# PKU-Alignment/SafeVLA

Hardware: AMD Instinct MI355X
Metric: env-steps/sec through PPO-Lagrangian update (higher is better)
Workload: dtype bf16

## Files before the change

safevla_amd/csrc/attn.hip:

```cpp
#include "attn_host.h"

#define HD 64
#define ATT_THREADS 256

struct AttnArgs {
    const bf16_t *Q, *K, *V; long ld;
    bf16_t* O; long ldo;
    float* LSE;
    const bf16_t* dO; long lddo;
    bf16_t *dQ, *dK, *dV; long ldd;
    const int* traj;
    const float* bias;
    const unsigned char* kvalid;
    int S, H, mask_mode;
    float scale;
    int kv_rows;
    int Sq;
    long ldq, lddq;
    float* Dws;
    DropCfg drop;
    int xcd_rows;
};

template <int SP, int THREADS = ATT_THREADS>
__device__ __forceinline__ void stage_head(bf16_t* dst, const bf16_t* src, long ld, int S, int tid) {
    constexpr int IT = SP * 8 / THREADS;
    u32x4 w[IT];
#pragma unroll
    for (int i = 0; i < IT; ++i) {
        const int q = tid + i * THREADS;
        const int row = q >> 3, c = q & 7;
        w[i] = u32x4{0, 0, 0, 0};
        if (row < S) w[i] = *(const u32x4*)(src + (size_t)row * ld + c * 8);
    }
#pragma unroll
    for (int i = 0; i < IT; ++i) {
        const int q = tid + i * THREADS;
        *(u32x4*)(dst + (q >> 3) * LDSROW + (((q & 7) ^ att_swz(q >> 3)) << 3)) = w[i];
    }
}

template <int NKT, bool GENERIC, int NW = 4, bool EXACT = false>
__device__ __forceinline__ void attn_fwd_kernel_body(AttnArgs p) {
    p.drop = drop_resolve(p.drop);
    extern __shared__ __attribute__((aligned(16))) char smem[];
    constexpr int SP = NKT * 16;
    bf16_t* Ks = (bf16_t*)smem;
    bf16_t* Vs = Ks + SP * LDSROW;
    int* traj_s = (int*)(Vs + SP * LDSROW);
    unsigned char* kv_s = (unsigned char*)(traj_s + SP);
    const int tid = threadIdx.x, lane = tid & 63, wid = tid >> 6;
    const int r = blockIdx.x / p.H, h = blockIdx.x % p.H;
    const size_t tok0 = (size_t)r * p.kv_rows, mtok0 = (size_t)r * p.S;
    const int S = p.S;
    stage_head<SP, NW * 64>(Ks, p.K + tok0 * p.ld + h * HD, p.ld, S, tid);
    stage_head<SP, NW * 64>(Vs, p.V + tok0 * p.ld + h * HD, p.ld, S, tid);
    for (int i = tid; i < SP; i += NW * 64) {
        traj_s[i] = (p.traj && i < S) ? p.traj[mtok0 + i] : -1;
        kv_s[i] = (p.kvalid && i < S) ? p.kvalid[mtok0 + i] : 1;
    }
    const int ql = lane & 15, g = lane >> 4;
    const int Sq = p.Sq;
    const size_t qtok0 = (size_t)r * Sq;
    const int nqt = (Sq + 15) / 16;
    constexpr int MAXQT = (NKT + NW - 1) / NW;
    bf16x8 qall[MAXQT][2];
#pragma unroll
    for (int t = 0; t < MAXQT; ++t) {
        const int q = (wid + NW * t) * 16 + ql;
        const bool ok = q < Sq;
        const bf16_t* qp = p.Q + (qtok0 + (ok ? q : 0)) * p.ldq + h * HD + 8 * g;
        qall[t][0] = ok ? *(const bf16x8*)qp : bf16x8{0, 0, 0, 0, 0, 0, 0, 0};
        qall[t][1] = ok ? *(const bf16x8*)(qp + 32) : bf16x8{0, 0, 0, 0, 0, 0, 0, 0};
    }
    __syncthreads();
    const unsigned char* kvp = p.kvalid ? kv_s : nullptr;
    const RowBase Krow = att_row_base(Ks, lane);
    const TrBase Vtr = att_tr_base(Vs, lane);
#pragma unroll
    for (int t = 0; t < MAXQT; ++t) {
        const int qt = wid + NW * t;
        if (qt >= nqt) break;
        const int q = qt * 16 + ql;
        const bf16x8 qf[2] = {qall[t][0], qall[t][1]};
        float sc[NKT][4];
        float mx = -INFINITY;
        const float sl2 = p.scale * LOG2E;
#pragma unroll
        for (int kt = 0; kt < NKT; ++kt) {
            f32x4 a = {0.f, 0.f, 0.f, 0.f};
            if (EXACT || kt * 16 < S) {
                a = mfma16(lds_row8i(Krow.lo, kt * 16), qf[0], a);
                a = mfma16(lds_row8i(Krow.hi, kt * 16), qf[1], a);
            }
            if constexpr (GENERIC) {
#pragma unroll
                for (int e = 0; e < 4; ++e) {
                    const int key = kt * 16 + 4 * g + e;
                    float s = a[e] * p.scale;
                    if (p.bias && q < Sq && key < S) s += p.bias[((size_t)h * S + q) * S + key];
                    s *= LOG2E;
                    if (att_masked(p, q < Sq ? q : 0, key, traj_s, kvp)) s = -INFINITY;
                    sc[kt][e] = s;
                    mx = fmaxf(mx, s);
                }
            } else {
                const bool tail = EXACT ? kt >= NKT - 2 : (kt + 1) * 16 > S;
#pragma unroll
                for (int e = 0; e < 4; ++e) {
                    float s = a[e] * sl2;
                    if (tail && kt * 16 + 4 * g + e >= S) s = -INFINITY;
                    sc[kt][e] = s;
                    mx = fmaxf(mx, s);
                }
            }
        }
        mx = fmaxf(mx, __shfl_xor(mx, 16, 64));
        mx = fmaxf(mx, __shfl_xor(mx, 32, 64));
        if (mx == -INFINITY) mx = 0.f;
        float lsum = 0.f;
#pragma unroll
        for (int kt = 0; kt < NKT; ++kt)
#pragma unroll
            for (int e = 0; e < 4; ++e) { sc[kt][e] = __builtin_amdgcn_exp2f(sc[kt][e] - mx); lsum += sc[kt][e]; }
        lsum += __shfl_xor(lsum, 16, 64);
        lsum += __shfl_xor(lsum, 32, 64);
        if (p.drop.thr) {
            const unsigned long long rb = att_drop_row(p.S, p.H, r, h, q < Sq ? q : 0);
#pragma unroll
            for (int kt = 0; kt < NKT; ++kt) {
                const unsigned keep = drop_keep4(p.drop, rb + kt * 16 + 4 * g);
#pragma unroll
                for (int e = 0; e < 4; ++e) if (!((keep >> e) & 1u)) sc[kt][e] = 0.f;
            }
        }
        f32x4 o[4];
#pragma unroll
        for (int dt = 0; dt < 4; ++dt) o[dt] = f32x4{0.f, 0.f, 0.f, 0.f};
#pragma unroll
        for (int u = 0; u < NKT / 2; ++u) {
            if (EXACT || u * 32 < S) {
                const float pv[8] = {sc[2 * u][0], sc[2 * u][1], sc[2 * u][2], sc[2 * u][3],
                                     sc[2 * u + 1][0], sc[2 * u + 1][1], sc[2 * u + 1][2], sc[2 * u + 1][3]};
                const bf16x8 pa = pack8(pv);
#pragma unroll
                for (int dt = 0; dt < 4; ++dt)
                    o[dt] = mfma16(lds_tr8i(Vtr.d[dt], 32 * u, 32 * u + 16), pa, o[dt]);
            }
        }
        const float inv = lsum > 0.f ? p.drop.scale / lsum : 0.f;
        if (q < Sq) {
#pragma unroll
            for (int dt = 0; dt < 4; ++dt) {
                const u32x2 w = {pack_bf2(o[dt][0] * inv, o[dt][1] * inv), pack_bf2(o[dt][2] * inv, o[dt][3] * inv)};
                *(u32x2*)(p.O + (qtok0 + q) * p.ldo + h * HD + dt * 16 + 4 * g) = w;
            }
        }
        if (p.LSE && g == 0 && q < Sq) p.LSE[((size_t)r * p.H + h) * Sq + q] = (mx + __log2f(lsum)) * LN2;
    }
}

__device__ __forceinline__ void att_xcd_item(const AttnArgs& p, int item, int nitems, int& r, int& h) {
    if (!p.xcd_rows) return;
    const int x = item & 7, j = item >> 3, nfull = (nitems / 64) * 8;
    if ((j >> 3) * 8 + x < nfull) { r = (j >> 3) * 8 + x; h = j & 7; }
}
struct AttDrop {
    unsigned a0;
    unsigned hb;
    bool wrap;
    unsigned long long p0;
};
__device__ __forceinline__ AttDrop att_drop_head(const AttnArgs& p, int r, int h) {
    AttDrop d;
    d.p0 = att_drop_row(p.S, p.H, r, h, 0) >> 1;
    d.a0 = (unsigned)d.p0 * 0x9E3779B1u;
    d.hb = ((unsigned)(d.p0 >> 32) * 0x85EBCA77u) ^ p.drop.key;
    d.wrap = (unsigned)d.p0 > 0xFFFF0000u;
    return d;
}

template <int NKT>
__device__ __forceinline__ void attn_fwd_persist_kernel_body(AttnArgs p, int nitems) {
    p.drop = drop_resolve(p.drop);
    extern __shared__ __attribute__((aligned(16))) char smem[];
    constexpr int SP = NKT * 16, IT = SP * 8 / ATT_THREADS, MAXQT = (NKT + 3) / 4;
    bf16_t* Ks = (bf16_t*)smem;
    bf16_t* Vs = Ks + SP * LDSROW;
    const int tid = threadIdx.x, lane = tid & 63, wid = tid >> 6;
    const int ql = lane & 15, g = lane >> 4;
    const int S = p.S, Sq = p.Sq, nqt = (Sq + 15) / 16;
    u32x4 kreg[IT], vreg[IT];
    bf16x8 qreg[MAXQT][2];
    auto fetch = [&](int item) {
        int r = item / p.H, h = item % p.H;
        att_xcd_item(p, item, nitems, r, h);
        const bf16_t* kp = p.K + (size_t)r * p.kv_rows * p.ld + h * HD;
        const bf16_t* vp = p.V + (size_t)r * p.kv_rows * p.ld + h * HD;
#pragma unroll
        for (int i = 0; i < IT; ++i) {
            const int q = tid + i * ATT_THREADS, row = q >> 3, c = q & 7;
            kreg[i] = u32x4{0, 0, 0, 0}; vreg[i] = u32x4{0, 0, 0, 0};
            if (row < S) {
                kreg[i] = *(const u32x4*)(kp + (size_t)row * p.ld + c * 8);
                vreg[i] = *(const u32x4*)(vp + (size_t)row * p.ld + c * 8);
            }
        }
#pragma unroll
        for (int t = 0; t < MAXQT; ++t) {
            const int q = (wid + 4 * t) * 16 + ql;
            const bool ok = q < Sq;
            const bf16_t* qp = p.Q + ((size_t)r * Sq + (ok ? q : 0)) * p.ldq + h * HD + 8 * g;
            qreg[t][0] = ok ? *(const bf16x8*)qp : bf16x8{0, 0, 0, 0, 0, 0, 0, 0};
            qreg[t][1] = ok ? *(const bf16x8*)(qp + 32) : bf16x8{0, 0, 0, 0, 0, 0, 0, 0};
        }
    };
    int item = blockIdx.x;
    if (item >= nitems) return;
    fetch(item);
    const RowBase Krow = att_row_base(Ks, lane);
    const TrBase Vtr = att_tr_base(Vs, lane);
    const float sl2 = p.scale * LOG2E;
    for (; item < nitems; item += gridDim.x) {
        int r = item / p.H, h = item % p.H;
        att_xcd_item(p, item, nitems, r, h);
        const size_t qtok0 = (size_t)r * Sq;
        __syncthreads();
#pragma unroll
        for (int i = 0; i < IT; ++i) {
            const int q = tid + i * ATT_THREADS;
            const int off = (q >> 3) * LDSROW + (((q & 7) ^ att_swz(q >> 3)) << 3);
            *(u32x4*)(Ks + off) = kreg[i];
            *(u32x4*)(Vs + off) = vreg[i];
        }
        bf16x8 qcur[MAXQT][2];
#pragma unroll
        for (int t = 0; t < MAXQT; ++t) { qcur[t][0] = qreg[t][0]; qcur[t][1] = qreg[t][1]; }
        __syncthreads();
        if (item + (int)gridDim.x < nitems) fetch(item + gridDim.x);
#pragma unroll
        for (int t = 0; t < MAXQT; ++t) {
            const int qt = wid + 4 * t;
            if (qt >= nqt) break;
            const int q = qt * 16 + ql;
            f32x4 sc[NKT];
            f32x4 mx4 = {-INFINITY, -INFINITY, -INFINITY, -INFINITY};
#pragma unroll
            for (int kt = 0; kt < NKT; ++kt) {
                f32x4 a = {0.f, 0.f, 0.f, 0.f};
                a = mfma16(lds_row8i(Krow.lo, kt * 16), qcur[t][0], a);
                a = mfma16(lds_row8i(Krow.hi, kt * 16), qcur[t][1], a);
                if (kt >= NKT - 2) {
#pragma unroll
                    for (int e = 0; e < 4; ++e)
                        if (kt * 16 + 4 * g + e >= S) a[e] = -INFINITY;
                }
                sc[kt] = a;
                mx4 = __builtin_elementwise_max(mx4, a);
            }
            float mx = fmaxf(fmaxf(mx4[0], mx4[1]), fmaxf(mx4[2], mx4[3]));
            mx = fmaxf(mx, __shfl_xor(mx, 16, 64));
            mx = fmaxf(mx, __shfl_xor(mx, 32, 64));
            const float nm = -mx * sl2;
            const f32x4 nm4 = {nm, nm, nm, nm}, sl4 = {sl2, sl2, sl2, sl2};
            f32x4 ls4 = {0.f, 0.f, 0.f, 0.f};
#pragma unroll
            for (int kt = 0; kt < NKT; ++kt) {
                const f32x4 x = sc[kt] * sl4 + nm4;
#pragma unroll
                for (int e = 0; e < 4; ++e) sc[kt][e] = __builtin_amdgcn_exp2f(x[e]);
                ls4 += sc[kt];
            }
            float lsum = (ls4[0] + ls4[1]) + (ls4[2] + ls4[3]);
            lsum += __shfl_xor(lsum, 16, 64);
            lsum += __shfl_xor(lsum, 32, 64);
            if (p.drop.thr) {
                const AttDrop dh = att_drop_head(p, r, h);
                const int S4 = (S + 3) & ~3, hS = S4 >> 1;
                const unsigned thr = p.drop.thr;
                if (!dh.wrap) {
                    const unsigned al = dh.a0 + (unsigned)(ql * hS + 2 * g) * 0x9E3779B1u;
                    const unsigned uq = (unsigned)(qt * 16 * hS) * 0x9E3779B1u;
#pragma unroll
                    for (int kt = 0; kt < NKT; ++kt) {
                        const unsigned ub = uq + (unsigned)(kt * 8) * 0x9E3779B1u;
                        const unsigned r0 = drop_mix((al + ub) ^ dh.hb), r1 = drop_mix((al + ub + 0x9E3779B1u) ^ dh.hb);
                        if ((r0 & 0xffffu) < thr) sc[kt][0] = 0.f;
                        if ((r0 >> 16) < thr) sc[kt][1] = 0.f;
                        if ((r1 & 0xffffu) < thr) sc[kt][2] = 0.f;
                        if ((r1 >> 16) < thr) sc[kt][3] = 0.f;
                    }
                } else {
                    const unsigned long long rb = att_drop_row(p.S, p.H, r, h, q < Sq ? q : 0);
#pragma unroll
                    for (int kt = 0; kt < NKT; ++kt) {
                        const unsigned keep = drop_keep4(p.drop, rb + kt * 16 + 4 * g);
#pragma unroll
                        for (int e = 0; e < 4; ++e) if (!((keep >> e) & 1u)) sc[kt][e] = 0.f;
                    }
                }
            }
            f32x4 o[4];
#pragma unroll
            for (int dt = 0; dt < 4; ++dt) o[dt] = f32x4{0.f, 0.f, 0.f, 0.f};
#pragma unroll
            for (int u = 0; u < NKT / 2; ++u) {
                const float pv[8] = {sc[2 * u][0], sc[2 * u][1], sc[2 * u][2], sc[2 * u][3],
                                     sc[2 * u + 1][0], sc[2 * u + 1][1], sc[2 * u + 1][2], sc[2 * u + 1][3]};
                const bf16x8 pa = pack8(pv);
#pragma unroll
                for (int dt = 0; dt < 4; ++dt)
                    o[dt] = mfma16(lds_tr8i(Vtr.d[dt], 32 * u, 32 * u + 16), pa, o[dt]);
            }
            const float inv = lsum > 0.f ? p.drop.scale / lsum : 0.f;
            if (q < Sq) {
#pragma unroll
                for (int dt = 0; dt < 4; ++dt) {
                    const u32x2 w = {pack_bf2(o[dt][0] * inv, o[dt][1] * inv), pack_bf2(o[dt][2] * inv, o[dt][3] * inv)};
                    *(u32x2*)(p.O + (qtok0 + q) * p.ldo + h * HD + dt * 16 + 4 * g) = w;
                }
            }
            if (p.LSE && g == 0 && q < Sq) p.LSE[((size_t)r * p.H + h) * Sq + q] = (mx * sl2 + __log2f(lsum)) * LN2;
        }
    }
}


template <int NKT, bool GENERIC>
__global__ void __launch_bounds__(ATT_THREADS) attn_bwd_dq_kernel(AttnArgs p) {
    p.drop = drop_resolve(p.drop);
    extern __shared__ __attribute__((aligned(16))) char smem[];
    constexpr int SP = NKT * 16;
    bf16_t* Ks = (bf16_t*)smem;
    bf16_t* Vs = Ks + SP * LDSROW;
    int* traj_s = (int*)(Vs + SP * LDSROW);
    unsigned char* kv_s = (unsigned char*)(traj_s + SP);
    const int tid = threadIdx.x, lane = tid & 63, wid = tid >> 6;
    const int r = blockIdx.x / p.H, h = blockIdx.x % p.H;
    const size_t tok0 = (size_t)r * p.S;
    const int S = p.S;
    stage_head<SP>(Ks, p.K + tok0 * p.ld + h * HD, p.ld, S, tid);
    stage_head<SP>(Vs, p.V + tok0 * p.ld + h * HD, p.ld, S, tid);
    for (int i = tid; i < SP; i += ATT_THREADS) {
        traj_s[i] = (p.traj && i < S) ? p.traj[tok0 + i] : -1;
        kv_s[i] = (p.kvalid && i < S) ? p.kvalid[tok0 + i] : 1;
    }
    const int ql = lane & 15, g = lane >> 4;
    const int Sq = p.Sq;
    const size_t qtok0 = (size_t)r * Sq;
    constexpr int MAXQT = (NKT + 3) / 4;
    bf16x8 qall[MAXQT][4];
    float dall[MAXQT], lall[MAXQT];
#pragma unroll
    for (int t = 0; t < MAXQT; ++t) {
        const int q = (wid + 4 * t) * 16 + ql;
        const bool qok = q < Sq;
        const bf16_t* qp = p.Q + (qtok0 + (qok ? q : 0)) * p.ldq + h * HD + 8 * g;
        const bf16_t* gp = p.dO + (qtok0 + (qok ? q : 0)) * p.lddo + h * HD + 8 * g;
        const bf16_t* op = p.O + (qtok0 + (qok ? q : 0)) * p.ldo + h * HD + 8 * g;
        qall[t][0] = gld8(qp, qok); qall[t][1] = gld8(qp + 32, qok);
        qall[t][2] = gld8(gp, qok); qall[t][3] = gld8(gp + 32, qok);
        dall[t] = dot8(qall[t][2], gld8(op, qok)) + dot8(qall[t][3], gld8(op + 32, qok));
        lall[t] = qok ? p.LSE[((size_t)r * p.H + h) * Sq + q] : INFINITY;
    }
    __syncthreads();
    const unsigned char* kvp = p.kvalid ? kv_s : nullptr;
    const RowBase Krow = att_row_base(Ks, lane), Vrow = att_row_base(Vs, lane);
    const TrBase Ktr = att_tr_base(Ks, lane);
    const int ntile = (Sq + 15) / 16;
#pragma unroll
    for (int t = 0; t < MAXQT; ++t) {
        const int qt = wid + 4 * t;
        if (qt >= ntile) break;
        const int q = qt * 16 + ql;
        const bool qok = q < Sq;
        const bf16x8 qf0 = qall[t][0], qf1 = qall[t][1], gf0 = qall[t][2], gf1 = qall[t][3];
        float D_q = dall[t];
        D_q += __shfl_xor(D_q, 16, 64);
        D_q += __shfl_xor(D_q, 32, 64);
        const float lse_q = lall[t];
        const float sl2 = p.scale * LOG2E, lse2_q = lse_q * LOG2E;
        f32x4 dq[4];
#pragma unroll
        for (int dt = 0; dt < 4; ++dt) dq[dt] = f32x4{0.f, 0.f, 0.f, 0.f};
#pragma unroll
        for (int u = 0; u < NKT / 2; ++u) {
            if (u * 32 < S) {
                float dsv[8];
#pragma unroll
                for (int e2 = 0; e2 < 2; ++e2) {
                    const int kt = 2 * u + e2;
                    f32x4 s = {0.f, 0.f, 0.f, 0.f}, dp = {0.f, 0.f, 0.f, 0.f};
                    s = mfma16(lds_row8i(Krow.lo, kt * 16), qf0, s);
                    s = mfma16(lds_row8i(Krow.hi, kt * 16), qf1, s);
                    dp = mfma16(lds_row8i(Vrow.lo, kt * 16), gf0, dp);
                    dp = mfma16(lds_row8i(Vrow.hi, kt * 16), gf1, dp);
                    const unsigned dkeep = p.drop.thr ? drop_keep4(p.drop, att_drop_row(p.S, p.H, r, h, qok ? q : 0) + kt * 16 + 4 * g) : 0xfu;
                    if constexpr (GENERIC) {
#pragma unroll
                        for (int e = 0; e < 4; ++e) {
                            const int key = kt * 16 + 4 * g + e;
                            float sv = s[e] * p.scale;
                            if (p.bias && qok && key < S) sv += p.bias[((size_t)h * S + q) * S + key];
                            const bool mk = !qok || att_masked(p, qok ? q : 0, key, traj_s, kvp);
                            const float pr = mk ? 0.f : __expf(sv - lse_q);
                            dsv[e2 * 4 + e] = pr * (((dkeep >> e) & 1u ? dp[e] * p.drop.scale : 0.f) - D_q) * p.scale;
                        }
                    } else {
#pragma unroll
                        for (int e = 0; e < 4; ++e)
                            dsv[e2 * 4 + e] = __builtin_amdgcn_exp2f(s[e] * sl2 - lse2_q) * (((dkeep >> e) & 1u ? dp[e] * p.drop.scale : 0.f) - D_q) * p.scale;
                    }
                }
                const bf16x8 da = pack8(dsv);
#pragma unroll
                for (int dt = 0; dt < 4; ++dt)
                    dq[dt] = mfma16(lds_tr8i(Ktr.d[dt], 32 * u, 32 * u + 16), da, dq[dt]);
            }
        }
        if (qok) {
#pragma unroll
            for (int dt = 0; dt < 4; ++dt) {
                const u32x2 w = {pack_bf2(dq[dt][0], dq[dt][1]), pack_bf2(dq[dt][2], dq[dt][3])};
                *(u32x2*)(p.dQ + (qtok0 + q) * p.lddq + h * HD + dt * 16 + 4 * g) = w;
            }
        }
    }
}

template <int NKT, bool GENERIC>
__global__ void __launch_bounds__(ATT_THREADS, NKT <= 12 ? 3 : 1) attn_bwd_dkv_kernel(AttnArgs p) {
    p.drop = drop_resolve(p.drop);
    extern __shared__ __attribute__((aligned(16))) char smem[];
    constexpr int SP = NKT * 16;
    bf16_t* Qs = (bf16_t*)smem;
    bf16_t* Gs = Qs + SP * LDSROW;
    float* lse_s = (float*)(Gs + SP * LDSROW);
    float* D_s = lse_s + SP;
    int* traj_s = (int*)(D_s + SP);
    unsigned char* kv_s = (unsigned char*)(traj_s + SP);
    const int tid = threadIdx.x, lane = tid & 63, wid = tid >> 6;
    const int r = blockIdx.x / p.H, h = blockIdx.x % p.H;
    const size_t tok0 = (size_t)r * p.S;
    const int S = p.S;
    constexpr int MAXKT = (NKT + 3) / 4;
    bf16x8 kvbuf[2][4];
    auto load_kv = [&](int t, bf16x8 (&dst)[4]) {
        const int keyl = (wid + 4 * t) * 16 + (lane & 15);
        const bool kok = keyl < S;
        const bf16_t* kp = p.K + (tok0 + (kok ? keyl : 0)) * p.ld + h * HD + 8 * (lane >> 4);
        const bf16_t* vp = p.V + (tok0 + (kok ? keyl : 0)) * p.ld + h * HD + 8 * (lane >> 4);
        dst[0] = gld8(kp, kok); dst[1] = gld8(kp + 32, kok);
        dst[2] = gld8(vp, kok); dst[3] = gld8(vp + 32, kok);
    };
    load_kv(0, kvbuf[0]);
    const int Sq = p.Sq;
    const size_t qtok0 = (size_t)r * Sq;
    stage_head<SP>(Qs, p.Q + qtok0 * p.ldq + h * HD, p.ldq, Sq, tid);
    stage_head<SP>(Gs, p.dO + qtok0 * p.lddo + h * HD, p.lddo, Sq, tid);
    for (int i = tid; i < SP; i += ATT_THREADS) {
        traj_s[i] = (p.traj && i < S) ? p.traj[tok0 + i] : -1;
        kv_s[i] = (p.kvalid && i < S) ? p.kvalid[tok0 + i] : 1;
        lse_s[i] = i < Sq ? p.LSE[((size_t)r * p.H + h) * Sq + i] * (GENERIC ? 1.f : LOG2E) : INFINITY;
    }
    {
        constexpr int IT = SP * 4 / ATT_THREADS;
        float part[IT];
#pragma unroll
        for (int i = 0; i < IT; ++i) {
            const int q = tid + i * ATT_THREADS;
            const int row = q >> 2, c = (q & 3) * 16;
            part[i] = 0.f;
            if (row < Sq) {
                const bf16_t* gp = p.dO + (qtok0 + row) * p.lddo + h * HD + c;
                const bf16_t* op = p.O + (qtok0 + row) * p.ldo + h * HD + c;
                part[i] = dot8(*(const bf16x8*)gp, *(const bf16x8*)op) + dot8(*(const bf16x8*)(gp + 8), *(const bf16x8*)(op + 8));
            }
        }
#pragma unroll
        for (int i = 0; i < IT; ++i) {
            float v = part[i];
            v += __shfl_xor(v, 1, 64);
            v += __shfl_xor(v, 2, 64);
            const int q = tid + i * ATT_THREADS;
            if ((q & 3) == 0) D_s[q >> 2] = v;
        }
    }
    __syncthreads();
    const unsigned char* kvp = p.kvalid ? kv_s : nullptr;
    const int ql = lane & 15, g = lane >> 4;
    const int ntile = (S + 15) / 16;
    const float sl2 = p.scale * LOG2E;
    const RowBase Qrow = att_row_base(Qs, lane), Grow = att_row_base(Gs, lane);
    const TrBase Qtr = att_tr_base(Qs, lane), Gtr = att_tr_base(Gs, lane);
#pragma unroll
    for (int t = 0; t < MAXKT; ++t) {
        const int kt = wid + 4 * t;
        if (kt >= ntile) break;
        const int keyl = kt * 16 + ql;
        const bool kok = keyl < S;
        if (t + 1 < MAXKT && kt + 4 < ntile) load_kv(t + 1, kvbuf[(t + 1) & 1]);
        const bf16x8 kf0 = kvbuf[t & 1][0], kf1 = kvbuf[t & 1][1], vf0 = kvbuf[t & 1][2], vf1 = kvbuf[t & 1][3];
        f32x4 dk[4], dv[4];
#pragma unroll
        for (int dt = 0; dt < 4; ++dt) { dk[dt] = f32x4{0.f, 0.f, 0.f, 0.f}; dv[dt] = f32x4{0.f, 0.f, 0.f, 0.f}; }
#pragma unroll
        for (int w = 0; w < NKT / 2; ++w) {
            if (w * 32 < Sq) {
                float pv[8], dsv[8];
#pragma unroll
                for (int e2 = 0; e2 < 2; ++e2) {
                    const int qt = 2 * w + e2;
                    f32x4 s = {0.f, 0.f, 0.f, 0.f}, dp = {0.f, 0.f, 0.f, 0.f};
                    s = mfma16(lds_row8i(Qrow.lo, qt * 16), kf0, s);
                    s = mfma16(lds_row8i(Qrow.hi, qt * 16), kf1, s);
                    dp = mfma16(lds_row8i(Grow.lo, qt * 16), vf0, dp);
                    dp = mfma16(lds_row8i(Grow.hi, qt * 16), vf1, dp);
                    if constexpr (GENERIC) {
#pragma unroll
                        for (int e = 0; e < 4; ++e) {
                            const int q = qt * 16 + 4 * g + e;
                            float sv = s[e] * p.scale;
                            if (p.bias && q < S && kok) sv += p.bias[((size_t)h * S + q) * S + keyl];
                            const bool mk = (q >= Sq) || att_masked(p, q < Sq ? q : 0, keyl, traj_s, kvp);
                            const float pr = mk ? 0.f : __expf(sv - lse_s[q]);
                            const bool kp = !p.drop.thr || att_keep1(p.drop, att_drop_row(p.S, p.H, r, h, q < Sq ? q : 0) + keyl);
                            pv[e2 * 4 + e] = kp ? pr * p.drop.scale : 0.f;
                            dsv[e2 * 4 + e] = pr * ((kp ? dp[e] * p.drop.scale : 0.f) - D_s[q]) * p.scale;
                        }
                    } else {
                        const f32x4 l4 = *(const f32x4*)(lse_s + 4 * g + qt * 16), d4 = *(const f32x4*)(D_s + 4 * g + qt * 16);
#pragma unroll
                        for (int e = 0; e < 4; ++e) {
                            const float pr = __builtin_amdgcn_exp2f(s[e] * sl2 - l4[e]);
                            const int q = qt * 16 + 4 * g + e;
                            const bool kp = !p.drop.thr || att_keep1(p.drop, att_drop_row(p.S, p.H, r, h, q < Sq ? q : 0) + keyl);
                            pv[e2 * 4 + e] = kp ? pr * p.drop.scale : 0.f;
                            dsv[e2 * 4 + e] = pr * ((kp ? dp[e] * p.drop.scale : 0.f) - d4[e]) * p.scale;
                        }
                    }
                }
                const bf16x8 pa = pack8(pv), da = pack8(dsv);
#pragma unroll
                for (int dt = 0; dt < 4; ++dt) {
                    dv[dt] = mfma16(lds_tr8i(Gtr.d[dt], 32 * w, 32 * w + 16), pa, dv[dt]);
                    dk[dt] = mfma16(lds_tr8i(Qtr.d[dt], 32 * w, 32 * w + 16), da, dk[dt]);
                }
            }
        }
        if (kok) {
#pragma unroll
            for (int dt = 0; dt < 4; ++dt) {
                const u32x2 wk = {pack_bf2(dk[dt][0], dk[dt][1]), pack_bf2(dk[dt][2], dk[dt][3])};
                const u32x2 wv = {pack_bf2(dv[dt][0], dv[dt][1]), pack_bf2(dv[dt][2], dv[dt][3])};
                *(u32x2*)(p.dK + (tok0 + keyl) * p.ldd + h * HD + dt * 16 + 4 * g) = wk;
                *(u32x2*)(p.dV + (tok0 + keyl) * p.ldd + h * HD + dt * 16 + 4 * g) = wv;
            }
        }
    }
}

template <int NKT>
__global__ void __launch_bounds__(ATT_THREADS, NKT <= 12 ? 3 : 2) attn_bwd_dq_exact_kernel(AttnArgs p) {
    p.drop = drop_resolve(p.drop);
    extern __shared__ __attribute__((aligned(16))) char smem[];
    constexpr int SP = NKT * 16, MAXQT = (NKT + 3) / 4;
    bf16_t* Ks = (bf16_t*)smem;
    bf16_t* Vs = Ks + SP * LDSROW;
    const int tid = threadIdx.x, lane = tid & 63, wid = tid >> 6;
    const int r = blockIdx.x / p.H, h = blockIdx.x % p.H;
    const size_t tok0 = (size_t)r * p.S;
    const int S = p.S, Sq = p.Sq;
    stage_head<SP>(Ks, p.K + tok0 * p.ld + h * HD, p.ld, S, tid);
    stage_head<SP>(Vs, p.V + tok0 * p.ld + h * HD, p.ld, S, tid);
    const int ql = lane & 15, g = lane >> 4;
    const size_t qtok0 = (size_t)r * Sq;
    bf16x8 qall[MAXQT][4];
    float dall[MAXQT], lall[MAXQT];
#pragma unroll
    for (int t = 0; t < MAXQT; ++t) {
        const int q = (wid + 4 * t) * 16 + ql;
        const bool qok = q < Sq;
        const bf16_t* qp = p.Q + (qtok0 + (qok ? q : 0)) * p.ldq + h * HD + 8 * g;
        const bf16_t* gp = p.dO + (qtok0 + (qok ? q : 0)) * p.lddo + h * HD + 8 * g;
        const bf16_t* op = p.O + (qtok0 + (qok ? q : 0)) * p.ldo + h * HD + 8 * g;
        qall[t][0] = gld8(qp, qok); qall[t][1] = gld8(qp + 32, qok);
        qall[t][2] = gld8(gp, qok); qall[t][3] = gld8(gp + 32, qok);
        dall[t] = dot8(qall[t][2], gld8(op, qok)) + dot8(qall[t][3], gld8(op + 32, qok));
        lall[t] = qok ? p.LSE[((size_t)r * p.H + h) * Sq + q] * LOG2E : INFINITY;
    }
    __syncthreads();
    const RowBase Krow = att_row_base(Ks, lane), Vrow = att_row_base(Vs, lane);
    const TrBase Ktr = att_tr_base(Ks, lane);
    const int ntile = (Sq + 15) / 16;
    const float sl2 = p.scale * LOG2E;
    const f32x4 sl4 = {sl2, sl2, sl2, sl2}, sc4 = {p.scale, p.scale, p.scale, p.scale};
#pragma unroll
    for (int t = 0; t < MAXQT; ++t) {
        const int qt = wid + 4 * t;
        if (qt < ntile) {
            const int q = qt * 16 + ql;
            const bool qok = q < Sq;
            float D_q = dall[t];
            D_q += __shfl_xor(D_q, 16, 64);
            D_q += __shfl_xor(D_q, 32, 64);
            if (p.Dws && g == 0 && qok) p.Dws[((size_t)r * p.H + h) * Sq + q] = D_q;
            const f32x4 nl4 = {-lall[t], -lall[t], -lall[t], -lall[t]}, nd4 = {-D_q, -D_q, -D_q, -D_q};
            const unsigned long long drow = att_drop_row(p.S, p.H, r, h, qok ? q : 0);
            f32x4 dq[4];
#pragma unroll
            for (int dt = 0; dt < 4; ++dt) dq[dt] = f32x4{0.f, 0.f, 0.f, 0.f};
#pragma unroll 2
            for (int u = 0; u < NKT / 2; ++u) {
                const int off = u * 32 * LDSROW;
                float dsv[8];
#pragma unroll
                for (int e2 = 0; e2 < 2; ++e2) {
                    const int o2 = off + e2 * 16 * LDSROW;
                    f32x4 sv = {0.f, 0.f, 0.f, 0.f}, dp = {0.f, 0.f, 0.f, 0.f};
                    sv = mfma16(*(const bf16x8*)(Krow.lo + o2), qall[t][0], sv);
                    sv = mfma16(*(const bf16x8*)(Krow.hi + o2), qall[t][1], sv);
                    dp = mfma16(*(const bf16x8*)(Vrow.lo + o2), qall[t][2], dp);
// ... 502 lines not shown
```

Baseline: 8062.

## Restructure attention forward: fused packed dropout, V prefetch, permlane reductions

Splits the forward attention body into QK and PV helpers. The PV step double-buffers the V fragment LDS reads one step ahead, applies dropout on packed bf16 pairs with u16 SIMD ops instead of per-element branches, and adds scheduling group barriers to interleave MFMA with VALU and LDS work. Row max and sum reductions now use permlane16/32 swaps instead of shuffles, and global address offsets are hoisted out of the loops. This adds inline asm and scheduler hints that may not suit every NKT configuration, and assumes bf16 multiplied by 0 or 1 as integers matches the old masking.

```diff
diff --git a/safevla_amd/csrc/attn.hip b/safevla_amd/csrc/attn.hip
--- a/safevla_amd/csrc/attn.hip
+++ b/safevla_amd/csrc/attn.hip
@@ -180,6 +180,73 @@
     return d;
 }
 
+
+template <class F>
+__device__ __forceinline__ float att_query_reduce(float v, F f) {
+    const unsigned x = __float_as_uint(v);
+    const auto a = __builtin_amdgcn_permlane16_swap(x, x, false, false);
+    const unsigned y = __float_as_uint(f(__uint_as_float(a[0]), __uint_as_float(a[1])));
+    const auto b = __builtin_amdgcn_permlane32_swap(y, y, false, false);
+    return f(__uint_as_float(b[0]), __uint_as_float(b[1]));
+}
+template <int NKT>
+__device__ __forceinline__ void att_fwd_qk(const RowBase& Krow, bf16x8 q0, bf16x8 q1, int S, int g, f32x4 (&sc)[NKT]) {
+#pragma unroll
+    for (int kt = 0; kt < NKT; ++kt) {
+        f32x4 a = {0.f, 0.f, 0.f, 0.f};
+        a = mfma16(lds_row8i(Krow.lo, kt * 16), q0, a);
+        a = mfma16(lds_row8i(Krow.hi, kt * 16), q1, a);
+        if (kt >= NKT - 2) {
+#pragma unroll
+            for (int e = 0; e < 4; ++e)
+                if (kt * 16 + 4 * g + e >= S) a[e] = -INFINITY;
+        }
+        sc[kt] = a;
+    }
+}
+__device__ __forceinline__ unsigned att_drop_pair(unsigned w, unsigned r, unsigned thm1x2) {
+    unsigned d, k, out;
+    asm("v_pk_sub_u16 %0, %1, %2 clamp" : "=v"(d) : "v"(r), "s"(thm1x2));
+    asm("v_pk_min_u16 %0, %1, %2" : "=v"(k) : "v"(d), "s"(0x00010001u));
+    asm("v_pk_mul_lo_u16 %0, %1, %2" : "=v"(out) : "v"(w), "v"(k));
+    return out;
+}
+template <int NKT, int DROP>
+__device__ __forceinline__ void att_fwd_pv(const TrBase& Vtr, const f32x4 (&pr)[NKT], f32x4 (&o)[4], unsigned thm1x2, unsigned a, unsigned hb, unsigned key,
+                                           unsigned long long pair0) {
+    bf16x8 vf[2][4];
+#pragma unroll
+    for (int dt = 0; dt < 4; ++dt) vf[0][dt] = lds_tr8i(Vtr.d[dt], 0, 16);
+#pragma unroll
+    for (int u = 0; u < NKT / 2; ++u) {
+        u32x4 w;
+        if (u + 1 < NKT / 2) {
+#pragma unroll
+            for (int dt = 0; dt < 4; ++dt) vf[(u + 1) & 1][dt] = lds_tr8i(Vtr.d[dt], 32 * u + 32, 32 * u + 48);
+        }
+#pragma unroll
+        for (int e2 = 0; e2 < 2; ++e2) {
+            const int kt = 2 * u + e2;
+            unsigned w0 = pack_bf2(pr[kt][0], pr[kt][1]), w1 = pack_bf2(pr[kt][2], pr[kt][3]);
+            if constexpr (DROP == 1) {
+                const unsigned x = a + (unsigned)(kt * 8) * 0x9E3779B1u;
+                w0 = att_drop_pair(w0, drop_mix(x ^ hb), thm1x2);
+                w1 = att_drop_pair(w1, drop_mix((x + 0x9E3779B1u) ^ hb), thm1x2);
+            } else if constexpr (DROP == 2) {
+                w0 = att_drop_pair(w0, drop_bits(key, pair0 + kt * 8), thm1x2);
+                w1 = att_drop_pair(w1, drop_bits(key, pair0 + kt * 8 + 1), thm1x2);
+            }
+            w[2 * e2] = w0; w[2 * e2 + 1] = w1;
+        }
+        const bf16x8 pa = __builtin_bit_cast(bf16x8, w);
+#pragma unroll
+        for (int dt = 0; dt < 4; ++dt) o[dt] = mfma16(vf[u & 1][dt], pa, o[dt]);
+        __builtin_amdgcn_sched_group_barrier(0x100, 8, 0);
+        __builtin_amdgcn_sched_group_barrier(0x2, 64, 0);
+        __builtin_amdgcn_sched_group_barrier(0x8, 4, 0);
+    }
+}
+
 template <int NKT>
 __device__ __forceinline__ void attn_fwd_persist_kernel_body(AttnArgs p, int nitems) {
     p.drop = drop_resolve(p.drop);
@@ -192,6 +259,8 @@
     const int S = p.S, Sq = p.Sq, nqt = (Sq + 15) / 16;
     u32x4 kreg[IT], vreg[IT];
     bf16x8 qreg[MAXQT][2];
+    const size_t kvoff = (size_t)(tid >> 3) * p.ld + (tid & 7) * 8;
+    const size_t qoff = (size_t)(wid * 16 + ql) * p.ldq + 8 * g, ooff = (size_t)(wid * 16 + ql) * p.ldo + 4 * g;
     auto fetch = [&](int item) {
         int r = item / p.H, h = item % p.H;
         att_xcd_item(p, item, nitems, r, h);
@@ -199,20 +268,20 @@
         const bf16_t* vp = p.V + (size_t)r * p.kv_rows * p.ld + h * HD;
 #pragma unroll
         for (int i = 0; i < IT; ++i) {
-            const int q = tid + i * ATT_THREADS, row = q >> 3, c = q & 7;
             kreg[i] = u32x4{0, 0, 0, 0}; vreg[i] = u32x4{0, 0, 0, 0};
-            if (row < S) {
-                kreg[i] = *(const u32x4*)(kp + (size_t)row * p.ld + c * 8);
-                vreg[i] = *(const u32x4*)(vp + (size_t)row * p.ld + c * 8);
-            }
-        }
+            if (i < IT - 1 || (tid >> 3) + i * 32 < S) {
+                kreg[i] = *(const u32x4*)(kp + (size_t)i * 32 * p.ld + kvoff);
+                vreg[i] = *(const u32x4*)(vp + (size_t)i * 32 * p.ld + kvoff);
+            }
+        }
+        const bf16_t* qp = p.Q + (size_t)r * Sq * p.ldq + h * HD;
 #pragma unroll
         for (int t = 0; t < MAXQT; ++t) {
-            const int q = (wid + 4 * t) * 16 + ql;
-            const bool ok = q < Sq;
-            const bf16_t* qp = p.Q + ((size_t)r * Sq + (ok ? q : 0)) * p.ldq + h * HD + 8 * g;
-            qreg[t][0] = ok ? *(const bf16x8*)qp : bf16x8{0, 0, 0, 0, 0, 0, 0, 0};
-            qreg[t][1] = ok ? *(const bf16x8*)(qp + 32) : bf16x8{0, 0, 0, 0, 0, 0, 0, 0};
+            qreg[t][0] = qreg[t][1] = bf16x8{0, 0, 0, 0, 0, 0, 0, 0};
+            if ((wid + 4 * t) * 16 + ql < Sq) {
+                qreg[t][0] = *(const bf16x8*)(qp + (size_t)t * 64 * p.ldq + qoff);
+                qreg[t][1] = *(const bf16x8*)(qp + (size_t)t * 64 * p.ldq + qoff + 32);
+            }
         }
     };
     int item = blockIdx.x;
@@ -244,23 +313,11 @@
             if (qt >= nqt) break;
             const int q = qt * 16 + ql;
             f32x4 sc[NKT];
-            f32x4 mx4 = {-INFINITY, -INFINITY, -INFINITY, -INFINITY};
-#pragma unroll
-            for (int kt = 0; kt < NKT; ++kt) {
-                f32x4 a = {0.f, 0.f, 0.f, 0.f};
-                a = mfma16(lds_row8i(Krow.lo, kt * 16), qcur[t][0], a);
-                a = mfma16(lds_row8i(Krow.hi, kt * 16), qcur[t][1], a);
-                if (kt >= NKT - 2) {
-#pragma unroll
-                    for (int e = 0; e < 4; ++e)
-                        if (kt * 16 + 4 * g + e >= S) a[e] = -INFINITY;
-                }
-                sc[kt] = a;
-                mx4 = __builtin_elementwise_max(mx4, a);
-            }
-            float mx = fmaxf(fmaxf(mx4[0], mx4[1]), fmaxf(mx4[2], mx4[3]));
-            mx = fmaxf(mx, __shfl_xor(mx, 16, 64));
-            mx = fmaxf(mx, __shfl_xor(mx, 32, 64));
+            att_fwd_qk<NKT>(Krow, qcur[t][0], qcur[t][1], S, g, sc);
+            f32x4 mx4 = sc[0];
+#pragma unroll
+            for (int kt = 1; kt < NKT; ++kt) mx4 = __builtin_elementwise_max(mx4, sc[kt]);
+            const float mx = att_query_reduce(fmaxf(fmaxf(mx4[0], mx4[1]), fmaxf(mx4[2], mx4[3])), [](float a, float b) { return fmaxf(a, b); });
             const float nm = -mx * sl2;
             const f32x4 nm4 = {nm, nm, nm, nm}, sl4 = {sl2, sl2, sl2, sl2};
             f32x4 ls4 = {0.f, 0.f, 0.f, 0.f};
@@ -271,53 +328,31 @@
                 for (int e = 0; e < 4; ++e) sc[kt][e] = __builtin_amdgcn_exp2f(x[e]);
                 ls4 += sc[kt];
             }
-            float lsum = (ls4[0] + ls4[1]) + (ls4[2] + ls4[3]);
-            lsum += __shfl_xor(lsum, 16, 64);
-            lsum += __shfl_xor(lsum, 32, 64);
+            const float lsum = att_query_reduce((ls4[0] + ls4[1]) + (ls4[2] + ls4[3]), [](float a, float b) { return a + b; });
+            f32x4 o[4];
+#pragma unroll
+            for (int dt = 0; dt < 4; ++dt) o[dt] = f32x4{0.f, 0.f, 0.f, 0.f};
             if (p.drop.thr) {
                 const AttDrop dh = att_drop_head(p, r, h);
                 const int S4 = (S + 3) & ~3, hS = S4 >> 1;
-                const unsigned thr = p.drop.thr;
+                const unsigned thm1x2 = (p.drop.thr - 1u) * 0x10001u;
                 if (!dh.wrap) {
-                    const unsigned al = dh.a0 + (unsigned)(ql * hS + 2 * g) * 0x9E3779B1u;
-                    const unsigned uq = (unsigned)(qt * 16 * hS) * 0x9E3779B1u;
-#pragma unroll
-                    for (int kt = 0; kt < NKT; ++kt) {
-                        const unsigned ub = uq + (unsigned)(kt * 8) * 0x9E3779B1u;
-                        const unsigned r0 = drop_mix((al + ub) ^ dh.hb), r1 = drop_mix((al + ub + 0x9E3779B1u) ^ dh.hb);
-                        if ((r0 & 0xffffu) < thr) sc[kt][0] = 0.f;
-                        if ((r0 >> 16) < thr) sc[kt][1] = 0.f;
-                        if ((r1 & 0xffffu) < thr) sc[kt][2] = 0.f;
-                        if ((r1 >> 16) < thr) sc[kt][3] = 0.f;
-                    }
+                    const unsigned a = dh.a0 + (unsigned)(ql * hS + 2 * g) * 0x9E3779B1u + (unsigned)(qt * 16 * hS) * 0x9E3779B1u;
+                    att_fwd_pv<NKT, 1>(Vtr, sc, o, thm1x2, a, dh.hb, 0u, 0ull);
                 } else {
                     const unsigned long long rb = att_drop_row(p.S, p.H, r, h, q < Sq ? q : 0);
-#pragma unroll
-                    for (int kt = 0; kt < NKT; ++kt) {
-                        const unsigned keep = drop_keep4(p.drop, rb + kt * 16 + 4 * g);
-#pragma unroll
-                        for (int e = 0; e < 4; ++e) if (!((keep >> e) & 1u)) sc[kt][e] = 0.f;
-                    }
-                }
-            }
-            f32x4 o[4];
-#pragma unroll
-            for (int dt = 0; dt < 4; ++dt) o[dt] = f32x4{0.f, 0.f, 0.f, 0.f};
-#pragma unroll
-            for (int u = 0; u < NKT / 2; ++u) {
-                const float pv[8] = {sc[2 * u][0], sc[2 * u][1], sc[2 * u][2], sc[2 * u][3],
-                                     sc[2 * u + 1][0], sc[2 * u + 1][1], sc[2 * u + 1][2], sc[2 * u + 1][3]};
-                const bf16x8 pa = pack8(pv);
-#pragma unroll
-                for (int dt = 0; dt < 4; ++dt)
-                    o[dt] = mfma16(lds_tr8i(Vtr.d[dt], 32 * u, 32 * u + 16), pa, o[dt]);
+                    att_fwd_pv<NKT, 2>(Vtr, sc, o, thm1x2, 0u, 0u, p.drop.key, (rb >> 1) + 2 * g);
+                }
+            } else {
+                att_fwd_pv<NKT, 0>(Vtr, sc, o, 0u, 0u, 0u, 0u, 0ull);
             }
             const float inv = lsum > 0.f ? p.drop.scale / lsum : 0.f;
             if (q < Sq) {
+                bf16_t* op = p.O + (qtok0 + (size_t)t * 64) * p.ldo + h * HD + ooff;
 #pragma unroll
                 for (int dt = 0; dt < 4; ++dt) {
                     const u32x2 w = {pack_bf2(o[dt][0] * inv, o[dt][1] * inv), pack_bf2(o[dt][2] * inv, o[dt][3] * inv)};
-                    *(u32x2*)(p.O + (qtok0 + q) * p.ldo + h * HD + dt * 16 + 4 * g) = w;
+                    *(u32x2*)(op + dt * 16) = w;
                 }
             }
             if (p.LSE && g == 0 && q < Sq) p.LSE[((size_t)r * p.H + h) * Sq + q] = (mx * sl2 + __log2f(lsum)) * LN2;
```

After: 8112 (median of 6 runs). No clear change (+0.6%).
